# privacy-scaling-explorations/snark-verifier

Measured on AMD Instinct MI355X. Metric: BN254 G1 MSM points/sec at 2^20, higher is better.
Workload: dtype i32x9 (254-bit Montgomery Fq as 9 x 29-bit limbs on the integer VALU); 1 GPU; BN254 G1 Pippenger MSM, 2^20 random points/scalars per GPU, inputs resident in HBM, affine result (configs[1]); points_per_gpu=1048576, points_per_kernel_launch=1048576, window_bits=default, msms_in_flight=264

## Files before the change

snark-verifier_amd/csrc/msm_api.hip:

```cpp
#include <stdlib.h>
#include <algorithm>
#include "ctx.hpp"
#include "../../include/snarkv_pallas.h"

namespace snarkv {

bool pip_chunk_pipeline(size_t n, int window_bits, bool is_lane, size_t* chunk) {
  const size_t c = (size_t)1 << 20;
  const char* e = getenv("SNARKV_PIP_SPLIT");
  const int mode = e ? atoi(e) : 1;
  const size_t min_chunks = mode == 2 ? 2 : 3;
  if (chunk) *chunk = c;
  return SNARKV_CHUNK_PIPELINE && mode != 0 && (n + c - 1) / c >= min_chunks && window_bits == 0 && !is_lane;
}

int launch_msm_pippenger_auto(snarkv_ctx* ctx, const void* d_s, const void* d_p, size_t n, int window_bits, void* d_out,
                              bool partial_out) {
  size_t kChunk = 0;
  const bool split = pip_chunk_pipeline(n, window_bits, ctx->is_lane, &kChunk);
  const size_t chunks = (n + kChunk - 1) / kChunk;
  ctx->last_split_workers = 0;
  ctx->last_many_jobs = 0;
  if (!split) return launch_msm_pippenger(ctx, d_s, d_p, n, window_bits, d_out, partial_out);
  SNARKV_TRY(ctx_lanes(ctx));
  const bool tm = ctx->stage_timing;
  if (tm && !ctx->ev_ready) {
    for (int i = 0; i <= SNARKV_PIP_STAGES; ++i) SNARKV_HIP(hipEventCreate(&ctx->ev[i]));
    ctx->ev_ready = true;
  }
  if (tm) SNARKV_HIP(hipEventRecord(ctx->ev[0], ctx->stream));
  uint32_t c = 0, windows = 0, bpw = 0;
  SNARKV_TRY(pip_geometry(kChunk, 0, &c, &windows, &bpw));
  const size_t nb = (size_t)windows * bpw, grid_bytes = nb * SNARKV_G1_PARTIAL_BYTES;
  const int kWorkers = 2;
  void *grid[3], *tmp[3];
  bool started[3] = {false, false, false};
  for (int w = 0; w < kWorkers; ++w) {
    SNARKV_TRY(ctx_reserve(ctx->sub[w], SLOT_MGPU_GRID, grid_bytes, &grid[w]));
    SNARKV_TRY(ctx_reserve(ctx->sub[w], SLOT_MGPU_RECV, grid_bytes, &tmp[w]));
  }
  SNARKV_TRY(ctx_lanes_fork(ctx));
  for (size_t k = 0; k < chunks; ++k) {
    size_t lo = k * kChunk, len = std::min(kChunk, n - lo);
    int w = (int)(k % kWorkers);
    snarkv_ctx* lane = ctx->sub[w];
    lane->mont = ctx->mont;
    lane->stage_timing = tm;
    SNARKV_TRY(launch_msm_pippenger(lane, (const char*)d_s + 32 * lo, (const char*)d_p + 64 * lo, len, (int)c, nullptr, false,
                                    started[w] ? tmp[w] : grid[w]));
    if (started[w]) SNARKV_TRY(launch_buckets_add(lane, grid[w], tmp[w], nb));
    started[w] = true;
  }
  for (int w = 0; w < kWorkers; ++w) ctx->sub[w]->stage_timing = false;
  SNARKV_TRY(ctx_lanes_join(ctx));
  for (int w = 1; w < kWorkers; ++w)
    if (started[w]) SNARKV_TRY(launch_buckets_add(ctx, grid[0], grid[w], nb));
  void* d_part;
  SNARKV_TRY(ctx_reserve(ctx, SLOT_SPLIT_PARTIALS, SNARKV_G1_PARTIAL_BYTES, &d_part));
  ctx->last_split_workers = kWorkers;
  int rc = SNARKV_OK;
  if (partial_out) {
    rc = launch_buckets_reduce(ctx, grid[0], c, 0, windows, d_out);
  } else {
    rc = launch_buckets_reduce(ctx, grid[0], c, 0, windows, d_part);
    if (rc == SNARKV_OK) rc = launch_fold_partials(ctx, d_part, 1, d_out, false);
  }
  if (tm && rc == SNARKV_OK) SNARKV_HIP(hipEventRecord(ctx->ev[SNARKV_PIP_STAGES - 1], ctx->stream));
  return rc;
}

int launch_msm_pippenger_many(snarkv_ctx* ctx, size_t count, const void* const* d_s, const void* const* d_p,
                              const size_t* n, int window_bits, void* d_out, bool partial_out, hipEvent_t* ready) {
  const size_t ostride = partial_out ? SNARKV_G1_PARTIAL_BYTES : 64;
  ctx->last_many_jobs = 0;
  ctx->last_split_workers = 0;
  if (count == 0) return SNARKV_OK;
  uint32_t c0 = 0, w0 = 0, b0 = 0;
  bool uniform = true, large = false;
  size_t nmax = 0, sig = count * 1000003u + (size_t)(uint32_t)window_bits;
  for (size_t i = 0; i < count; ++i) {
    if (n[i] == 0) return SNARKV_ERR_EMPTY;
    uint32_t c, w, b;
    SNARKV_TRY(pip_geometry(n[i], window_bits, &c, &w, &b));
    if (i == 0) c0 = c, w0 = w, b0 = b;
    uniform = uniform && c == c0;
    large = large || pip_chunk_pipeline(n[i], window_bits, false, nullptr);
    nmax = std::max(nmax, n[i]);
    sig = sig * 31 + n[i];
  }
  const char* em = getenv("SNARKV_MANY_MODE");
  if (count == 1 || large || (em && atoi(em) == 0) || ctx->is_lane) {
    for (size_t i = 0; i < count; ++i) {
      if (ready) SNARKV_HIP(hipStreamWaitEvent(ctx->stream, ready[i], 0));
      SNARKV_TRY(launch_msm_pippenger_auto(ctx, d_s[i], d_p[i], n[i], window_bits, (uint8_t*)d_out + ostride * i, partial_out));
    }
    return SNARKV_OK;
  }
  const size_t per_job = nmax * 600 + (size_t)w0 * b0 * SNARKV_G1_PARTIAL_BYTES * 2 + (1u << 20);
  size_t G = std::min<size_t>(count, SNARKV_MANY_MAX_JOBS);
  G = std::max<size_t>(1, std::min<size_t>(G, ((size_t)48 << 30) / per_job));
  if (const char* eg = getenv("SNARKV_MANY_JOBS")) G = std::max<size_t>(1, std::min<size_t>(G, (size_t)atoi(eg)));
  const size_t rounds = (count + G - 1) / G;
  G = (count + rounds - 1) / rounds;
  SNARKV_TRY(ctx_lanes(ctx));
  while ((size_t)ctx->njobs < G) {
    snarkv_ctx* j = nullptr;
    SNARKV_TRY(SNARKV_API(ctx_create)(ctx->device, (void*)ctx->stream, &j));
    j->is_lane = true;
    j->throughput_mode = true;
    SNARKV_HIP(hipEventCreateWithFlags(&j->sorted_ev, hipEventDisableTiming));
    j->sorted_ev_ready = true;
    ctx->jobs[ctx->njobs++] = j;
  }
  if (!ctx->hi_ready) {
    int least = 0, greatest = 0;
    SNARKV_HIP(hipDeviceGetStreamPriorityRange(&least, &greatest));
    for (int i = 0; i < 2; ++i) SNARKV_HIP(hipStreamCreateWithPriority(&ctx->hi_stream[i], hipStreamNonBlocking, greatest));
    for (int i = 0; i < 2; ++i) SNARKV_HIP(hipEventCreateWithFlags(&ctx->many_ev[i], hipEventDisableTiming));
    ctx->hi_ready = true;
  }
  const bool tm = ctx->stage_timing;
  if (tm && !ctx->ev_ready) {
    for (int i = 0; i <= SNARKV_PIP_STAGES; ++i) SNARKV_HIP(hipEventCreate(&ctx->ev[i]));
    ctx->ev_ready = true;
  }
  if (sig != ctx->many_sig) {
    SNARKV_HIP(hipDeviceSynchronize());
    ctx->many_sig = sig;
  }
  hipStream_t S[3] = {ctx->stream, ctx->sub[0]->stream, ctx->sub[1]->stream};
  constexpr int nS = 3;
  auto join_and_fork = [&]() -> int {
    for (int k = 0; k < 2; ++k) {
      SNARKV_HIP(hipEventRecord(ctx->many_ev[k], ctx->hi_stream[k]));
      SNARKV_HIP(hipStreamWaitEvent(ctx->stream, ctx->many_ev[k], 0));
    }
    for (int k = 0; k + 1 < nS; ++k) {
      SNARKV_HIP(hipEventRecord(ctx->sub_ev[k], S[k + 1]));
      SNARKV_HIP(hipStreamWaitEvent(ctx->stream, ctx->sub_ev[k], 0));
    }
    SNARKV_HIP(hipEventRecord(ctx->sub_ev[4], ctx->stream));
    for (int k = 0; k < 2; ++k) SNARKV_HIP(hipStreamWaitEvent(ctx->hi_stream[k], ctx->sub_ev[4], 0));
    for (int k = 0; k + 1 < nS; ++k) SNARKV_HIP(hipStreamWaitEvent(S[k + 1], ctx->sub_ev[4], 0));
    return SNARKV_OK;
  };
  void* d_grids = nullptr;
  const size_t grid_bytes = (size_t)w0 * b0 * SNARKV_G1_PARTIAL_BYTES;
  if (uniform) SNARKV_TRY(ctx_reserve(ctx, SLOT_MGPU_GRID, grid_bytes * G, &d_grids));
  if (tm) SNARKV_HIP(hipEventRecord(ctx->ev[0], ctx->stream));
  SNARKV_TRY(join_and_fork());
  for (size_t lo = 0; lo < count; lo += G) {
    const size_t hi = std::min(count, lo + G);
    const bool last = hi == count;
    for (size_t i = lo; i < hi; ++i) {
      snarkv_ctx* job = ctx->jobs[i - lo];
      job->mont = ctx->mont;
      job->stage_timing = tm && last;
      void* grid = uniform ? (uint8_t*)d_grids + grid_bytes * (i - lo) : nullptr;
      hipStream_t sa = ctx->hi_stream[(i - lo) % 2], sb = S[(i - lo) % nS];
      if (ready) SNARKV_HIP(hipStreamWaitEvent(sa, ready[i], 0));
      SNARKV_TRY(launch_msm_pippenger_phases(job, sa, PIP_PHASE_SORT, d_s[i], d_p[i], n[i], window_bits, nullptr, false,
                                             nullptr, grid));
      SNARKV_HIP(hipEventRecord(job->sorted_ev, sa));
      SNARKV_HIP(hipStreamWaitEvent(sb, job->sorted_ev, 0));
      SNARKV_TRY(launch_msm_pippenger_phases(job, sb, PIP_PHASE_ACC, d_s[i], d_p[i], n[i], window_bits, nullptr, false,
                                             nullptr, grid));
      if (!uniform)
        SNARKV_TRY(launch_msm_pippenger_phases(job, sb, PIP_PHASE_TAIL, d_s[i], d_p[i], n[i], window_bits,
                                               (uint8_t*)d_out + ostride * i, partial_out, nullptr, nullptr));
      job->stage_timing = false;
    }
    SNARKV_TRY(join_and_fork());
    if (uniform) {
      SNARKV_TRY(launch_buckets_reduce_many(ctx, ctx->stream, d_grids, c0, w0, (uint32_t)(hi - lo),
                                            (uint8_t*)d_out + ostride * lo, partial_out));
      if (!last) SNARKV_TRY(join_and_fork());
    }
    if (last) ctx->last_many_jobs = (int)(hi - lo);
  }
  if (tm) SNARKV_HIP(hipEventRecord(ctx->ev[SNARKV_PIP_STAGES - 1], ctx->stream));
  return SNARKV_OK;
// ... 63 lines not shown
```

snark-verifier_amd/csrc/msm_pippenger.hip:

```cpp
#include <stdlib.h>
#include <string.h>
#include <algorithm>
#include <mutex>
#include <atomic>
#include "ctx.hpp"
#include "g1_29.h"
#include "fr29.h"
#ifndef SNARKV_GLV
#define SNARKV_GLV 1
#endif
#if SNARKV_GLV
#include "glv.h"
#endif

namespace snarkv {

#ifndef SNARKV_KRUN
#define SNARKV_KRUN 128
#endif
#ifndef SNARKV_KCHUNK
#define SNARKV_KCHUNK 8
#endif
#ifndef SNARKV_TILE_THREADS
#define SNARKV_TILE_THREADS 256
#endif
#ifndef SNARKV_SCATTER_ATTR
#define SNARKV_SCATTER_ATTR __attribute__((amdgpu_waves_per_eu(5)))
#endif
#ifndef SNARKV_L2_THREADS
#define SNARKV_L2_THREADS 512
#endif
#ifndef SNARKV_LEVEL2_ATTR
#define SNARKV_LEVEL2_ATTR
#endif
#ifndef SNARKV_PREP_THREADS
#define SNARKV_PREP_THREADS SNARKV_TILE_THREADS
#endif
#ifndef SNARKV_XCD_TILES
#define SNARKV_XCD_TILES 1
#endif
#ifndef SNARKV_TILE_BASE
#define SNARKV_TILE_BASE 2048
#endif
#ifndef SNARKV_ACC_WAVES
#define SNARKV_ACC_WAVES 3
#endif
#ifndef SNARKV_BPRIO
#define SNARKV_BPRIO 3
#endif
#define SNARKV_RAISE_PRIO() __builtin_amdgcn_s_setprio(SNARKV_BPRIO)

constexpr int kHalves = SNARKV_GLV ? 2 : 1;
constexpr int kDigitWords = SNARKV_GLV ? 4 : 8;
constexpr int kDigitBits = 32 * kDigitWords;
constexpr int kRun = SNARKV_KRUN;
#ifndef SNARKV_KRUN_THROUGHPUT
#define SNARKV_KRUN_THROUGHPUT 128
#endif
constexpr int kRunThroughput = SNARKV_KRUN_THROUGHPUT;
constexpr int kChunk = SNARKV_KCHUNK;
constexpr uint32_t kSortCap = 7168;
constexpr uint32_t kSortTarget = 3072;
constexpr uint32_t kMaxKeys = 16384;

struct PipParams {
  uint32_t n;
  int c;
  int W;
  uint32_t B;
  uint32_t nb;
  int low_bits;
  uint32_t SB;
  uint32_t nkeys;
  uint32_t nblk;
  uint32_t tile;
  uint32_t mstride;
  uint32_t w0;
  uint32_t krun;
  uint32_t wper;
  uint32_t chunk_log2;
  uint32_t mont;
};

__device__ __forceinline__ uint32_t half_bits(const uint32_t (&k)[kDigitWords], int lo, int c) {
  if (lo >= kDigitBits) return 0;
  int word = lo >> 5, sh = lo & 31;
  uint32_t w0 = 0u, w1 = 0u;
#pragma unroll
  for (int i = 0; i < kDigitWords; ++i) {
    w0 = word == i ? k[i] : w0;
    if (i > 0) w1 = word == i - 1 ? k[i] : w1;
  }
  uint64_t v = ((uint64_t)w1 << 32) | w0;
  return (uint32_t)(v >> sh) & ((1u << c) - 1u);
}

template <class F>
__device__ __forceinline__ void for_each_digit(const uint32_t (&k)[kDigitWords], uint32_t sgn, const PipParams& p, F emit) {
  uint32_t carry = 0;
  for (int w = 0; w < p.W; ++w) {
    uint32_t raw = half_bits(k, w * p.c, p.c) + carry;
    uint32_t neg = raw > p.B ? 1u : 0u;
    uint32_t d = neg ? ((1u << p.c) - raw) : raw;
    carry = neg;
    if (d != 0) emit((uint32_t)w * p.SB + ((d - 1) >> p.low_bits), (uint32_t)w * p.B + d - 1, neg ^ sgn);
  }
}
template <class F>
__device__ __forceinline__ void digit_of_window(const uint32_t (&k)[kDigitWords], uint32_t sgn, const PipParams& p, int w,
                                                F emit) {
  uint32_t carry = 0;
  for (int j = w - 1; j >= 0; --j) {
    uint32_t b = half_bits(k, j * p.c, p.c);
    if (b != p.B) {
      carry = b > p.B ? 1u : 0u;
      break;
    }
  }
  uint32_t raw = half_bits(k, w * p.c, p.c) + carry;
  uint32_t neg = raw > p.B ? 1u : 0u;
  uint32_t d = neg ? ((1u << p.c) - raw) : raw;
  if (d != 0) emit((uint32_t)w * p.SB + ((d - 1) >> p.low_bits), (uint32_t)w * p.B + d - 1, neg ^ sgn);
}
__device__ __forceinline__ uint32_t load_digit_words(const uint32_t* src, uint32_t (&k)[kDigitWords]) {
#pragma unroll
  for (int j = 0; j < kDigitWords; ++j) k[j] = src[j];
#if SNARKV_GLV
  uint32_t sgn = k[3] >> 31;
  k[3] &= 0x7FFFFFFFu;
  return sgn;
#else
  return 0u;
#endif
}
__device__ __forceinline__ uint32_t load_digit_source(const uint4* __restrict__ src, size_t v, uint32_t (&k)[kDigitWords]) {
  const uint4* s = src + v * (kDigitWords / 4);
#pragma unroll
  for (int j = 0; j < kDigitWords / 4; ++j) {
    uint4 q = s[j];
    k[4 * j] = q.x;
    k[4 * j + 1] = q.y;
    k[4 * j + 2] = q.z;
    k[4 * j + 3] = q.w;
  }
#if SNARKV_GLV
  uint32_t sgn = k[3] >> 31;
  k[3] &= 0x7FFFFFFFu;
  return sgn;
#else
  return 0u;
#endif
}

__device__ __forceinline__ uint32_t xcd_tile(uint32_t b, uint32_t nblk) {
#if SNARKV_XCD_TILES
  return (nblk & 7u) == 0 ? (b & 7u) * (nblk >> 3) + (b >> 3) : b;
#else
  return b;
#endif
}

__global__ void __launch_bounds__(SNARKV_PREP_THREADS)
    k_prepare(const uint32_t* __restrict__ scalars, const uint32_t* __restrict__ points,
              G1Packed* __restrict__ pts, uint4* __restrict__ glv, PipParams p, uint32_t* __restrict__ M) {
  SNARKV_RAISE_PRIO();
  extern __shared__ uint32_t lds[];
  for (uint32_t k = threadIdx.x; k < p.nkeys; k += blockDim.x) lds[k] = 0u;
  __syncthreads();
  const uint32_t tile = xcd_tile(blockIdx.x, p.nblk);
  uint32_t lo = tile * p.tile;
  uint32_t hi = lo + p.tile < p.n ? lo + p.tile : p.n;
  for (uint32_t i = lo + threadIdx.x; i < hi; i += blockDim.x) {
    const uint4* s = reinterpret_cast<const uint4*>(points + (size_t)i * 16);
    uint32_t w[16];
#pragma unroll
    for (int j = 0; j < 4; ++j) {
      uint4 v = s[j];
      w[4 * j] = v.x;
      w[4 * j + 1] = v.y;
      w[4 * j + 2] = v.z;
      w[4 * j + 3] = v.w;
    }
    G1Affine29 a = g1a29_from_words(w, p.mont != 0);
    bool ident = g1a29_is_identity(a);
    pts[kHalves * (size_t)i] = g1a29_pack(a);
    const uint4* ks = reinterpret_cast<const uint4*>(scalars + (size_t)i * 8);
    uint4 k0 = ks[0], k1 = ks[1];
    uint32_t k[8] = {k0.x, k0.y, k0.z, k0.w, k1.x, k1.y, k1.z, k1.w}, o[8];
    if (p.mont) {
      uint32_t kc[8];
      fr_words_from_mont256(k, kc);
#pragma unroll
      for (int j = 0; j < 8; ++j) k[j] = kc[j];
    }
#if SNARKV_GLV
    constexpr int32_t bl[9] = SNARKV_GLV_BETA29_LIMBS;
    Fq29 beta;
#pragma unroll
    for (int j = 0; j < 9; ++j) beta.v[j] = bl[j];
    a.x = fq29_canon_of_product(fq29_mul(a.x, beta));
    pts[2 * (size_t)i + 1] = g1a29_pack(a);
    glv_decompose(k, o);
#else
#pragma unroll
    for (int j = 0; j < 8; ++j) o[j] = k[j];
#endif
    if (ident) {
#pragma unroll
      for (int j = 0; j < 8; ++j) o[j] = 0;
    }
    glv[2 * (size_t)i] = make_uint4(o[0], o[1], o[2], o[3]);
    glv[2 * (size_t)i + 1] = make_uint4(o[4], o[5], o[6], o[7]);
#pragma unroll
    for (int h = 0; h < kHalves; ++h) {
      uint32_t d[kDigitWords];
      uint32_t sgn = load_digit_words(o + h * kDigitWords, d);
      for_each_digit(d, sgn, p, [&](uint32_t key, uint32_t, uint32_t) { atomicAdd(&lds[key], 1u); });
    }
  }
  __syncthreads();
  for (uint32_t k = threadIdx.x; k < p.nkeys; k += blockDim.x) M[(size_t)k * p.mstride + tile] = lds[k];
  if (blockIdx.x == 0 && p.mstride > p.nblk)
    for (uint32_t k = threadIdx.x; k < p.nkeys; k += blockDim.x) M[(size_t)k * p.mstride + p.nblk] = 0u;
}

constexpr uint32_t kStageScalars = SNARKV_TILE_BASE;
constexpr uint32_t kStageItems = kStageScalars / SNARKV_TILE_THREADS;
static_assert(kStageScalars % SNARKV_TILE_THREADS == 0, "a staged tile gives every lane the same number of scalars");
__global__ void __launch_bounds__(SNARKV_TILE_THREADS) SNARKV_SCATTER_ATTR
    k_sort_scatter_staged(const uint4* __restrict__ glv, PipParams p, const uint32_t* __restrict__ M,
                          uint2* __restrict__ tmp) {
  SNARKV_RAISE_PRIO();
  extern __shared__ uint32_t lds[];
  uint32_t* gbase = lds;
  uint32_t* cnt = lds + p.SB;
  uint32_t* off = lds + 2 * p.SB;
  uint32_t* wsum = lds + 3 * p.SB;
  uint2* stage = reinterpret_cast<uint2*>(lds + 3 * p.SB + 16 + (p.SB & 1u));
  const uint32_t tid = threadIdx.x, lane = tid & 63u, wave = tid >> 6;
  const uint32_t tile = xcd_tile(blockIdx.x, p.nblk);
  const uint32_t lo = tile * kStageScalars;
  const uint32_t hi = lo + kStageScalars < p.n ? lo + kStageScalars : p.n;
  const uint32_t per = (p.SB + SNARKV_TILE_THREADS - 1) / SNARKV_TILE_THREADS;
  for (int w = 0; w < p.W; ++w) {
    for (uint32_t k = tid; k < p.SB; k += blockDim.x) {
      gbase[k] = M[((size_t)w * p.SB + k) * p.mstride + tile];
      cnt[k] = 0u;
    }
    __syncthreads();
    uint32_t ebkt[kStageItems * kHalves], erank[kStageItems * kHalves], eneg = 0u;
#pragma unroll
    for (uint32_t j = 0; j < kStageItems; ++j) {
      const uint32_t i = lo + tid + j * SNARKV_TILE_THREADS;
#pragma unroll
      for (uint32_t h = 0; h < (uint32_t)kHalves; ++h) {
        const uint32_t e = j * kHalves + h;
        ebkt[e] = 0xFFFFFFFFu;
        if (i < hi) {
          uint32_t d[kDigitWords];
          uint32_t sgn = load_digit_source(glv, (size_t)kHalves * i + h, d);
          digit_of_window(d, sgn, p, w, [&](uint32_t key, uint32_t bucket, uint32_t neg) {
            ebkt[e] = bucket - (uint32_t)w * p.B;
            eneg |= neg << e;
            erank[e] = atomicAdd(&cnt[key - (uint32_t)w * p.SB], 1u);
          });
        }
      }
    }
    __syncthreads();
    uint32_t mine = 0;
    for (uint32_t k = tid * per; k < (tid + 1) * per && k < p.SB; ++k) mine += cnt[k];
    uint32_t incl = mine;
#pragma unroll
    for (int d = 1; d < 64; d <<= 1) {
      uint32_t up = __shfl_up(incl, d, 64);
      if ((int)lane >= d) incl += up;
    }
    if (lane == 63) wsum[wave] = incl;
    __syncthreads();
    uint32_t run = incl - mine;
    for (uint32_t q = 0; q < wave; ++q) run += wsum[q];
    for (uint32_t k = tid * per; k < (tid + 1) * per && k < p.SB; ++k) {
      off[k] = run;
      run += cnt[k];
    }
    __syncthreads();
#pragma unroll
    for (uint32_t e = 0; e < kStageItems * kHalves; ++e)
      if (ebkt[e] != 0xFFFFFFFFu) {
        const uint32_t v = kHalves * (lo + tid + (e / kHalves) * SNARKV_TILE_THREADS) + (e % kHalves);
        stage[off[ebkt[e] >> p.low_bits] + erank[e]] = make_uint2(ebkt[e] + (uint32_t)w * p.B, v | (((eneg >> e) & 1u) << 31));
      }
    __syncthreads();
    const uint32_t total = off[p.SB - 1] + cnt[p.SB - 1];
    for (uint32_t idx = tid; idx < total; idx += blockDim.x) {
      const uint2 e = stage[idx];
      const uint32_t key = (e.x - (uint32_t)w * p.B) >> p.low_bits;
      tmp[gbase[key] + (idx - off[key])] = e;
    }
    __syncthreads();
  }
}

__global__ void __launch_bounds__(256) k_scan_local(uint32_t* __restrict__ data, uint32_t* __restrict__ blocksum,
                                                    uint32_t nb) {
  SNARKV_RAISE_PRIO();
  __shared__ uint32_t sh[256];
  uint32_t base = blockIdx.x * 1024 + threadIdx.x * 4;
  uint32_t v[4], s = 0;
#pragma unroll
  for (int j = 0; j < 4; ++j) {
    v[j] = (base + j < nb) ? data[base + j] : 0;
    s += v[j];
  }
  sh[threadIdx.x] = s;
  __syncthreads();
  for (uint32_t off = 1; off < 256; off <<= 1) {
    uint32_t t = (threadIdx.x >= off) ? sh[threadIdx.x - off] : 0;
    __syncthreads();
    sh[threadIdx.x] += t;
    __syncthreads();
  }
  uint32_t excl = sh[threadIdx.x] - s;
#pragma unroll
  for (int j = 0; j < 4; ++j) {
    if (base + j < nb) data[base + j] = excl;
    excl += v[j];
  }
  if (threadIdx.x == 255) blocksum[blockIdx.x] = sh[255];
}

__global__ void __launch_bounds__(1024) k_scan_blocksums(uint32_t* __restrict__ blocksum, uint32_t nblocks,
                                                         uint32_t* __restrict__ total_out) {
  SNARKV_RAISE_PRIO();
  __shared__ uint32_t sh[1024];
  __shared__ uint32_t running;
  if (threadIdx.x == 0) running = 0;
  __syncthreads();
  for (uint32_t base = 0; base < nblocks; base += 1024) {
    uint32_t idx = base + threadIdx.x;
    uint32_t v = idx < nblocks ? blocksum[idx] : 0;
    sh[threadIdx.x] = v;
    __syncthreads();
    for (uint32_t off = 1; off < 1024; off <<= 1) {
      uint32_t t = (threadIdx.x >= off) ? sh[threadIdx.x - off] : 0;
      __syncthreads();
      sh[threadIdx.x] += t;
      __syncthreads();
// ... 475 lines not shown
                     (uint32_t*)d_out64, partial_out ? 1 : 0, ctx->mont ? 1u : 0u);
  SNARKV_HIP(hipGetLastError());
  return SNARKV_OK;
}

static int default_window_bits(size_t n) {
  int best = 2;
  double best_cost = 0;
  for (int c = 2; c <= 22; ++c) {
    const int W = (kDigitBits + c - 1) / c;
    const int top = kDigitBits - 1 - (W - 1) * c;
    double cost = (double)kHalves * (double)n * W * 10.0 + (double)W * (double)(1u << (c - 1)) * 30.0;
    if (top < c - 3) cost *= 1.6;
    if (c == 2 || cost < best_cost) best = c, best_cost = cost;
  }
  return best;
}

static int balance_window_bits(int c) {
  int W = (kDigitBits + c - 1) / c;
  return (kDigitBits + W - 1) / W;
}

static uint32_t latency_run_length(uint64_t entries) {
  auto waves = [&](uint64_t run) { return (entries + 64 * run - 1) / (64 * run); };
  if (waves(16) <= 4608) return waves(16) >= 2048 ? 16u : 32u;
  if (waves(32) <= 4608) return 32u;
  return (uint32_t)kRun;
}
static_assert(kRun >= 32 && kRun <= (int)kMaxPiece && kRunThroughput >= 16 && kRunThroughput <= (int)kMaxPiece,
              "piece caps fit the schedule's LDS rows");

int launch_msm_pippenger(snarkv_ctx* ctx, const void* d_scalars, const void* d_points, size_t n, int window_bits,
                         void* d_out, bool partial_out, void* d_buckets_out) {
  return launch_msm_pippenger_phases(ctx, ctx->stream, PIP_PHASE_ALL, d_scalars, d_points, n, window_bits, d_out,
                                     partial_out, d_buckets_out, nullptr);
}

int launch_msm_pippenger_phases(snarkv_ctx* ctx, hipStream_t st, int phases, const void* d_scalars, const void* d_points,
                                size_t n, int window_bits, void* d_out, bool partial_out, void* d_buckets_out,
                                void* d_grid) {
  PipParams p;
  p.w0 = 0;
  p.wper = 0;
  p.chunk_log2 = (uint32_t)kLog2Chunk;
  p.mont = ctx->mont ? 1u : 0u;
  p.n = (uint32_t)n;
  p.c = window_bits > 0 ? window_bits : balance_window_bits(default_window_bits(n));
  if (p.c < 2) p.c = 2;
  if (p.c > 22) p.c = 22;
  p.W = (kDigitBits + p.c - 1) / p.c;
  p.B = 1u << (p.c - 1);
  p.nb = (uint32_t)p.W * p.B;
  int high = p.c - 1 > 10 ? p.c - 1 - 10 : 0;
  while (high < p.c - 1 && ((kHalves * n) >> (high + 1)) >= kSortTarget && ((uint64_t)p.W << (high + 1)) <= kMaxKeys) ++high;
  p.low_bits = (p.c - 1) - high;
  p.SB = p.B >> p.low_bits;
  p.nkeys = (uint32_t)p.W * p.SB;
  p.tile = SNARKV_TILE_BASE;
  static_assert(kStageItems * kHalves <= 32, "a staged lane keeps one sign bit per entry in a 32-bit word");
  const size_t lds_staged = ((size_t)3 * p.SB + 16 + (p.SB & 1u)) * 4 + (size_t)kStageScalars * kHalves * 8;
  p.nblk = (uint32_t)((n + p.tile - 1) / p.tile);
  p.mstride = p.nblk | 1u;
  uint64_t max_entries = (uint64_t)kHalves * (uint64_t)n * (uint64_t)p.W;
  if (n == 0 || max_entries >= 0xFFFFFFFFull || n >= 0x40000000ull) {
    set_last_error("pippenger: n=%zu out of range", n);
    return SNARKV_ERR_LENGTH;
  }
  if ((size_t)p.nkeys * 4 > 65536 || lds_staged > 96 * 1024) {
    set_last_error("pippenger: key table too large (nkeys=%u)", p.nkeys);
    return SNARKV_ERR_LENGTH;
  }
  p.krun = ctx->throughput_mode ? (uint32_t)kRunThroughput : latency_run_length(max_entries);
  const uint32_t max_pieces = (uint32_t)std::min<uint64_t>((uint64_t)p.nb + max_entries / p.krun, 0xFFFFFFFFull - 63);
  const uint32_t split_slots = (uint32_t)(max_entries / p.krun) + 1;
  const uint32_t nsb = (p.nb + kSchedBuckets - 1) / kSchedBuckets;
  const uint32_t hcount = sched_rows(p.krun) * nsb;
  const uint32_t hscan_blocks = (hcount + 1023) / 1024;
  uint32_t mcount = p.nkeys * p.mstride;
  uint32_t scan_blocks = (mcount + 1023) / 1024;
  uint32_t chunks_per_window = (p.B + kChunk - 1) / kChunk;
  uint32_t blocks_per_window = (chunks_per_window + 63) / 64;

  void *d_pts, *d_glv, *d_counts, *d_offsets, *d_M, *d_blocksum, *d_entries, *d_tmp, *d_pieces, *d_hist, *d_parts,
      *d_buckets, *d_wave, *d_shift, *d_misc, *d_lists;
  SNARKV_TRY(ctx_reserve(ctx, SLOT_POINTS_MONT, kHalves * n * sizeof(G1Packed), &d_pts));
  SNARKV_TRY(ctx_reserve(ctx, SLOT_GLV, n * 32, &d_glv));
  SNARKV_TRY(ctx_reserve(ctx, SLOT_COUNTS, (size_t)p.nb * 4, &d_counts));
  SNARKV_TRY(ctx_reserve(ctx, SLOT_OFFSETS, (size_t)p.nb * 4, &d_offsets));
  SNARKV_TRY(ctx_reserve(ctx, SLOT_CURSOR, (size_t)mcount * 4, &d_M));
  SNARKV_TRY(ctx_reserve(ctx, SLOT_BLOCKSUMS, (size_t)std::max(scan_blocks, hscan_blocks) * 4 + 64, &d_blocksum));
  SNARKV_TRY(ctx_reserve(ctx, SLOT_ENTRIES, max_entries * 8, &d_entries));
  SNARKV_TRY(ctx_reserve(ctx, SLOT_SORT_TMP, max_entries * 8, &d_tmp));
  SNARKV_TRY(ctx_reserve(ctx, SLOT_PIECES, (size_t)max_pieces * sizeof(uint4), &d_pieces));
  SNARKV_TRY(ctx_reserve(ctx, SLOT_PIECE_HIST, (size_t)hcount * 4, &d_hist));
  SNARKV_TRY(ctx_reserve(ctx, SLOT_SPLIT_PARTS, (size_t)split_slots * 2 * sizeof(G1Xyzz29), &d_parts));
  if (d_grid) d_buckets = d_grid;
  else SNARKV_TRY(ctx_reserve(ctx, SLOT_BUCKETS, (size_t)p.nb * sizeof(G1Xyzz29), &d_buckets));
  SNARKV_TRY(ctx_reserve(ctx, SLOT_CHUNK_PARTIALS, 2 * (size_t)blocks_per_window * p.W * sizeof(G1Xyzz29), &d_wave));
  SNARKV_TRY(ctx_reserve(ctx, SLOT_SHIFTED, (size_t)p.W * sizeof(G1Xyzz29), &d_shift));
  SNARKV_TRY(ctx_reserve(ctx, SLOT_MISC, 64, &d_misc));
  SNARKV_TRY(ctx_reserve(ctx, SLOT_FIX_LISTS, (size_t)p.nb * 3 * 4, &d_lists));
  uint32_t* d_total = (uint32_t*)d_misc;
  uint32_t* d_small = (uint32_t*)d_lists, *d_bigl = d_small + p.nb, *d_deg = d_bigl + p.nb;
  const uint32_t* d_npieces = (const uint32_t*)d_hist + (size_t)(p.krun + 1) * nsb;

  const bool tm = ctx->stage_timing && phases == PIP_PHASE_ALL;
  const bool tm_acc = ctx->stage_timing && phases == PIP_PHASE_ACC;
  int evi = 0;
#define STAGE_MARK()                                         \
  do {                                                       \
    if (tm) SNARKV_HIP(hipEventRecord(ctx->ev[evi++], st));  \
  } while (0)
  if ((tm || tm_acc) && !ctx->ev_ready) {
    for (int i = 0; i <= SNARKV_PIP_STAGES; ++i) SNARKV_HIP(hipEventCreate(&ctx->ev[i]));
    ctx->ev_ready = true;
  }
  STAGE_MARK();
  if (phases & PIP_PHASE_SORT) {
    hipLaunchKernelGGL(k_prepare, dim3(p.nblk), dim3(SNARKV_PREP_THREADS), (size_t)p.nkeys * 4, st, (const uint32_t*)d_scalars,
                       (const uint32_t*)d_points, (G1Packed*)d_pts, (uint4*)d_glv, p, (uint32_t*)d_M);
    STAGE_MARK();
    hipLaunchKernelGGL(k_scan_local, dim3(scan_blocks), dim3(256), 0, st, (uint32_t*)d_M, (uint32_t*)d_blocksum, mcount);
    hipLaunchKernelGGL(k_scan_blocksums, dim3(1), dim3(1024), 0, st, (uint32_t*)d_blocksum, scan_blocks, d_total);
    hipLaunchKernelGGL(k_scan_add, dim3(scan_blocks), dim3(256), 0, st, (uint32_t*)d_M, (const uint32_t*)d_blocksum,
                       mcount);
    STAGE_MARK();
    static std::atomic<uint64_t> attr_set{0};
    const uint64_t bit = 1ull << (ctx->device & 63);
    if (!(attr_set.load(std::memory_order_relaxed) & bit)) {
      SNARKV_HIP(hipFuncSetAttribute(reinterpret_cast<const void*>(k_sort_scatter_staged),
                                     hipFuncAttributeMaxDynamicSharedMemorySize, 96 * 1024));
      attr_set.fetch_or(bit, std::memory_order_relaxed);
    }
    hipLaunchKernelGGL(k_sort_scatter_staged, dim3(p.nblk), dim3(SNARKV_TILE_THREADS), lds_staged, st, (const uint4*)d_glv,
                       p, (const uint32_t*)d_M, (uint2*)d_tmp);
    const uint32_t nbins_l2 = 1u << p.low_bits;
    const size_t lds2 = ((size_t)nbins_l2 + SNARKV_L2_THREADS + 1) * 4 + (size_t)kSortCap * 8;
    hipLaunchKernelGGL(k_sort_level2, dim3(p.nkeys), dim3(SNARKV_L2_THREADS), lds2, st, (const uint2*)d_tmp, (const uint32_t*)d_M,
                       d_total, p, (uint2*)d_entries, (uint32_t*)d_counts, (uint32_t*)d_offsets);
    hipLaunchKernelGGL(k_piece_hist, dim3(nsb), dim3(256), 0, st, (const uint32_t*)d_counts, p, nsb, (uint32_t*)d_hist,
                       d_total);
    hipLaunchKernelGGL(k_scan_local, dim3(hscan_blocks), dim3(256), 0, st, (uint32_t*)d_hist, (uint32_t*)d_blocksum, hcount);
    hipLaunchKernelGGL(k_scan_blocksums, dim3(1), dim3(1024), 0, st, (uint32_t*)d_blocksum, hscan_blocks, d_total + 6);
    hipLaunchKernelGGL(k_scan_add, dim3(hscan_blocks), dim3(256), 0, st, (uint32_t*)d_hist, (const uint32_t*)d_blocksum,
                       hcount);
    hipLaunchKernelGGL(k_piece_emit, dim3(nsb), dim3(256), 0, st, (const uint32_t*)d_counts, (const uint32_t*)d_offsets, p,
                       nsb, (const uint32_t*)d_hist, split_slots, (uint4*)d_pieces, d_small, d_bigl);
  }
  STAGE_MARK();
  if (tm_acc) SNARKV_HIP(hipEventRecord(ctx->ev[3], st));
  if (phases & PIP_PHASE_ACC)
    hipLaunchKernelGGL(k_accumulate, dim3((max_pieces + 63) / 64), dim3(64), 0, st, (const uint4*)d_pieces, d_npieces,
                       (const uint32_t*)d_total, (const uint2*)d_entries, (const G1Packed*)d_pts, (G1Xyzz29*)d_buckets,
                       (G1Xyzz29*)d_parts, 2 * split_slots, d_total + 4, d_deg, p);
  STAGE_MARK();
  if (tm_acc) SNARKV_HIP(hipEventRecord(ctx->ev[4], st));
  if (phases & PIP_PHASE_ACC) {
    const uint64_t split_bound = std::min<uint64_t>(p.nb, max_entries / (p.krun + 1) + 1);
    const uint32_t fix_grid = (uint32_t)std::min<uint64_t>((split_bound + 255) / 256, kFixGrid);
    hipLaunchKernelGGL(k_fixup, dim3(fix_grid), dim3(256), 0, st, (const uint32_t*)d_counts, (const uint32_t*)d_offsets,
                       (const uint2*)d_entries, (const G1Packed*)d_pts, (const G1Xyzz29*)d_parts, split_slots,
                       (G1Xyzz29*)d_buckets, (const uint32_t*)d_hist, nsb, (const uint32_t*)d_total,
                       (const uint32_t*)d_small, (const uint32_t*)d_bigl, (const uint32_t*)d_deg, p);
    if (tm_acc) SNARKV_HIP(hipEventRecord(ctx->ev[5], st));
  }
  STAGE_MARK();
  if (d_buckets_out) {
    if (phases & PIP_PHASE_ACC)
      SNARKV_HIP(hipMemcpyAsync(d_buckets_out, d_buckets, (size_t)p.nb * sizeof(G1Xyzz29), hipMemcpyDeviceToDevice, st));
    SNARKV_HIP(hipGetLastError());
    return SNARKV_OK;
  }
  if (phases & PIP_PHASE_TAIL)
    hipLaunchKernelGGL(k_bucket_reduce, dim3(blocks_per_window * p.W), dim3(64), 0, st, (const G1Xyzz29*)d_buckets,
                       (G1Xyzz29*)d_wave, p, chunks_per_window, blocks_per_window);
  STAGE_MARK();
  if (phases & PIP_PHASE_TAIL)
    hipLaunchKernelGGL(k_shift_windows, dim3(p.W), dim3(64), 0, st, (const G1Xyzz29*)d_wave, (G1Xyzz29*)d_shift, p,
                       blocks_per_window);
  STAGE_MARK();
  if (phases & PIP_PHASE_TAIL)
    hipLaunchKernelGGL(k_final, dim3(1), dim3(64), 0, st, (const G1Xyzz29*)d_shift, (uint32_t)p.W, (uint32_t*)d_out,
                       partial_out ? 1 : 0, p.mont);
  STAGE_MARK();
#undef STAGE_MARK
  SNARKV_HIP(hipGetLastError());
  return SNARKV_OK;
}

int pip_geometry(size_t n_total, int window_bits, uint32_t* c, uint32_t* windows, uint32_t* buckets_per_window) {
  int cc = window_bits > 0 ? window_bits : balance_window_bits(default_window_bits(n_total));
  if (cc < 2) cc = 2;
  if (cc > 22) cc = 22;
  *c = (uint32_t)cc;
  *windows = (uint32_t)((kDigitBits + cc - 1) / cc);
  *buckets_per_window = 1u << (cc - 1);
  return SNARKV_OK;
}

__global__ void __launch_bounds__(256) k_buckets_add(G1Xyzz29* __restrict__ dst, const G1Xyzz29* __restrict__ src, uint32_t count) {
  SNARKV_RAISE_PRIO();
  uint32_t i = blockIdx.x * blockDim.x + threadIdx.x;
  if (i >= count) return;
  G1Xyzz29 a = dst[i];
  xyzz29_add_careful(a, src[i]);
  dst[i] = xyzz29_sanitize(a);
}

int launch_buckets_add(snarkv_ctx* ctx, void* d_dst, const void* d_src, size_t count) {
  hipLaunchKernelGGL(k_buckets_add, dim3((uint32_t)((count + 255) / 256)), dim3(256), 0, ctx->stream, (G1Xyzz29*)d_dst,
                     (const G1Xyzz29*)d_src, (uint32_t)count);
  SNARKV_HIP(hipGetLastError());
  return SNARKV_OK;
}

int launch_buckets_reduce(snarkv_ctx* ctx, const void* d_buckets, uint32_t c, uint32_t w0, uint32_t wcount,
                          void* d_partial) {
// ... 79 lines not shown
```

Baseline: 806.2 million points/s.

## Precompute signed window digits in prepare and store per-window digit planes

The prepare kernel now computes the signed-digit recoding once per scalar and writes a per-window plane of packed digit records (magnitude plus sign bit), with a specialised unrolled path for 16-bit windows. The scatter kernel then reads one small record per window instead of reloading the full GLV scalar halves and rescanning lower windows for the carry. This removes redundant digit recomputation and large scalar reloads in the sort scatter, at the cost of more global writes in prepare and a differently sized scratch buffer. The per-job memory estimate is raised to match.

```diff
diff --git a/snark-verifier_amd/csrc/msm_api.hip b/snark-verifier_amd/csrc/msm_api.hip
--- a/snark-verifier_amd/csrc/msm_api.hip
+++ b/snark-verifier_amd/csrc/msm_api.hip
@@ -96,7 +96,7 @@
     }
     return SNARKV_OK;
   }
-  const size_t per_job = nmax * 600 + (size_t)w0 * b0 * SNARKV_G1_PARTIAL_BYTES * 2 + (1u << 20);
+  const size_t per_job = nmax * 632 + (size_t)w0 * b0 * SNARKV_G1_PARTIAL_BYTES * 2 + (1u << 20);
   size_t G = std::min<size_t>(count, SNARKV_MANY_MAX_JOBS);
   G = std::max<size_t>(1, std::min<size_t>(G, ((size_t)48 << 30) / per_job));
   if (const char* eg = getenv("SNARKV_MANY_JOBS")) G = std::max<size_t>(1, std::min<size_t>(G, (size_t)atoi(eg)));
diff --git a/snark-verifier_amd/csrc/msm_pippenger.hip b/snark-verifier_amd/csrc/msm_pippenger.hip
--- a/snark-verifier_amd/csrc/msm_pippenger.hip
+++ b/snark-verifier_amd/csrc/msm_pippenger.hip
@@ -12,6 +12,7 @@
 #if SNARKV_GLV
 #include "glv.h"
 #endif
+#include "pip_digits.h"
 
 namespace snarkv {
 
@@ -82,46 +83,9 @@
   uint32_t mont;
 };
 
-__device__ __forceinline__ uint32_t half_bits(const uint32_t (&k)[kDigitWords], int lo, int c) {
-  if (lo >= kDigitBits) return 0;
-  int word = lo >> 5, sh = lo & 31;
-  uint32_t w0 = 0u, w1 = 0u;
-#pragma unroll
-  for (int i = 0; i < kDigitWords; ++i) {
-    w0 = word == i ? k[i] : w0;
-    if (i > 0) w1 = word == i - 1 ? k[i] : w1;
-  }
-  uint64_t v = ((uint64_t)w1 << 32) | w0;
-  return (uint32_t)(v >> sh) & ((1u << c) - 1u);
-}
-
-template <class F>
-__device__ __forceinline__ void for_each_digit(const uint32_t (&k)[kDigitWords], uint32_t sgn, const PipParams& p, F emit) {
-  uint32_t carry = 0;
-  for (int w = 0; w < p.W; ++w) {
-    uint32_t raw = half_bits(k, w * p.c, p.c) + carry;
-    uint32_t neg = raw > p.B ? 1u : 0u;
-    uint32_t d = neg ? ((1u << p.c) - raw) : raw;
-    carry = neg;
-    if (d != 0) emit((uint32_t)w * p.SB + ((d - 1) >> p.low_bits), (uint32_t)w * p.B + d - 1, neg ^ sgn);
-  }
-}
-template <class F>
-__device__ __forceinline__ void digit_of_window(const uint32_t (&k)[kDigitWords], uint32_t sgn, const PipParams& p, int w,
-                                                F emit) {
-  uint32_t carry = 0;
-  for (int j = w - 1; j >= 0; --j) {
-    uint32_t b = half_bits(k, j * p.c, p.c);
-    if (b != p.B) {
-      carry = b > p.B ? 1u : 0u;
-      break;
-    }
-  }
-  uint32_t raw = half_bits(k, w * p.c, p.c) + carry;
-  uint32_t neg = raw > p.B ? 1u : 0u;
-  uint32_t d = neg ? ((1u << p.c) - raw) : raw;
-  if (d != 0) emit((uint32_t)w * p.SB + ((d - 1) >> p.low_bits), (uint32_t)w * p.B + d - 1, neg ^ sgn);
-}
+#ifndef SNARKV_DIGITS_GENERIC
+#define SNARKV_DIGITS_GENERIC 0
+#endif
 __device__ __forceinline__ uint32_t load_digit_words(const uint32_t* src, uint32_t (&k)[kDigitWords]) {
 #pragma unroll
   for (int j = 0; j < kDigitWords; ++j) k[j] = src[j];
@@ -133,24 +97,15 @@
   return 0u;
 #endif
 }
-__device__ __forceinline__ uint32_t load_digit_source(const uint4* __restrict__ src, size_t v, uint32_t (&k)[kDigitWords]) {
-  const uint4* s = src + v * (kDigitWords / 4);
-#pragma unroll
-  for (int j = 0; j < kDigitWords / 4; ++j) {
-    uint4 q = s[j];
-    k[4 * j] = q.x;
-    k[4 * j + 1] = q.y;
-    k[4 * j + 2] = q.z;
-    k[4 * j + 3] = q.w;
-  }
 #if SNARKV_GLV
-  uint32_t sgn = k[3] >> 31;
-  k[3] &= 0x7FFFFFFFu;
-  return sgn;
+typedef uint2 DigitPair;
+__device__ __forceinline__ DigitPair digit_pair(const uint32_t (&r)[kHalves]) { return make_uint2(r[0], r[1]); }
+__device__ __forceinline__ void digit_unpair(DigitPair q, uint32_t (&r)[kHalves]) { r[0] = q.x, r[1] = q.y; }
 #else
-  return 0u;
-#endif
-}
+typedef uint32_t DigitPair;
+__device__ __forceinline__ DigitPair digit_pair(const uint32_t (&r)[kHalves]) { return r[0]; }
+__device__ __forceinline__ void digit_unpair(DigitPair q, uint32_t (&r)[kHalves]) { r[0] = q; }
+#endif
 
 __device__ __forceinline__ uint32_t xcd_tile(uint32_t b, uint32_t nblk) {
 #if SNARKV_XCD_TILES
@@ -162,7 +117,7 @@
 
 __global__ void __launch_bounds__(SNARKV_PREP_THREADS)
     k_prepare(const uint32_t* __restrict__ scalars, const uint32_t* __restrict__ points,
-              G1Packed* __restrict__ pts, uint4* __restrict__ glv, PipParams p, uint32_t* __restrict__ M) {
+              G1Packed* __restrict__ pts, uint32_t* __restrict__ dig, PipParams p, uint32_t* __restrict__ M) {
   SNARKV_RAISE_PRIO();
   extern __shared__ uint32_t lds[];
   for (uint32_t k = threadIdx.x; k < p.nkeys; k += blockDim.x) lds[k] = 0u;
@@ -209,13 +164,35 @@
 #pragma unroll
       for (int j = 0; j < 8; ++j) o[j] = 0;
     }
-    glv[2 * (size_t)i] = make_uint4(o[0], o[1], o[2], o[3]);
-    glv[2 * (size_t)i + 1] = make_uint4(o[4], o[5], o[6], o[7]);
+    uint32_t d[kHalves][kDigitWords], sgn[kHalves], carry[kHalves];
 #pragma unroll
     for (int h = 0; h < kHalves; ++h) {
-      uint32_t d[kDigitWords];
-      uint32_t sgn = load_digit_words(o + h * kDigitWords, d);
-      for_each_digit(d, sgn, p, [&](uint32_t key, uint32_t, uint32_t) { atomicAdd(&lds[key], 1u); });
+      sgn[h] = load_digit_words(o + h * kDigitWords, d[h]);
+      carry[h] = 0u;
+    }
+    DigitPair* plane = reinterpret_cast<DigitPair*>(dig) + i;
+    auto window = [&](int w, const uint32_t (&rec)[kHalves]) {
+      plane[(size_t)w * p.n] = digit_pair(rec);
+#pragma unroll
+      for (int h = 0; h < kHalves; ++h)
+        if (rec[h]) atomicAdd(&lds[(uint32_t)w * p.SB + (((rec[h] & kDigitMag) - 1u) >> p.low_bits)], 1u);
+    };
+    if (!SNARKV_DIGITS_GENERIC && p.c == 16) {
+#pragma unroll
+      for (int w = 0; w < kDigitBits / 16; ++w)
+        if (w < p.W) {
+          uint32_t rec[kHalves];
+#pragma unroll
+          for (int h = 0; h < kHalves; ++h) rec[h] = digit_step16<kDigitWords>(d[h], sgn[h], w, carry[h]);
+          window(w, rec);
+        }
+    } else {
+      for (int w = 0; w < p.W; ++w) {
+        uint32_t rec[kHalves];
+#pragma unroll
+        for (int h = 0; h < kHalves; ++h) rec[h] = digit_step<kDigitWords>(d[h], sgn[h], w, p.c, carry[h]);
+        window(w, rec);
+      }
     }
   }
   __syncthreads();
@@ -228,7 +205,7 @@
 constexpr uint32_t kStageItems = kStageScalars / SNARKV_TILE_THREADS;
 static_assert(kStageScalars % SNARKV_TILE_THREADS == 0, "a staged tile gives every lane the same number of scalars");
 __global__ void __launch_bounds__(SNARKV_TILE_THREADS) SNARKV_SCATTER_ATTR
-    k_sort_scatter_staged(const uint4* __restrict__ glv, PipParams p, const uint32_t* __restrict__ M,
+    k_sort_scatter_staged(const uint32_t* __restrict__ dig, PipParams p, const uint32_t* __restrict__ M,
                           uint2* __restrict__ tmp) {
   SNARKV_RAISE_PRIO();
   extern __shared__ uint32_t lds[];
@@ -249,21 +226,22 @@
     }
     __syncthreads();
     uint32_t ebkt[kStageItems * kHalves], erank[kStageItems * kHalves], eneg = 0u;
+    const DigitPair* plane = reinterpret_cast<const DigitPair*>(dig) + (size_t)w * p.n;
 #pragma unroll
     for (uint32_t j = 0; j < kStageItems; ++j) {
       const uint32_t i = lo + tid + j * SNARKV_TILE_THREADS;
+      uint32_t rec[kHalves];
+#pragma unroll
+      for (int h = 0; h < kHalves; ++h) rec[h] = 0u;
+      if (i < hi) digit_unpair(plane[i], rec);
 #pragma unroll
       for (uint32_t h = 0; h < (uint32_t)kHalves; ++h) {
         const uint32_t e = j * kHalves + h;
         ebkt[e] = 0xFFFFFFFFu;
-        if (i < hi) {
-          uint32_t d[kDigitWords];
-          uint32_t sgn = load_digit_source(glv, (size_t)kHalves * i + h, d);
-          digit_of_window(d, sgn, p, w, [&](uint32_t key, uint32_t bucket, uint32_t neg) {
-            ebkt[e] = bucket - (uint32_t)w * p.B;
-            eneg |= neg << e;
-            erank[e] = atomicAdd(&cnt[key - (uint32_t)w * p.SB], 1u);
-          });
+        if (rec[h]) {
+          ebkt[e] = (rec[h] & kDigitMag) - 1u;
+          eneg |= (rec[h] >> 31) << e;
+          erank[e] = atomicAdd(&cnt[ebkt[e] >> p.low_bits], 1u);
         }
       }
     }
@@ -905,10 +883,10 @@
   uint32_t chunks_per_window = (p.B + kChunk - 1) / kChunk;
   uint32_t blocks_per_window = (chunks_per_window + 63) / 64;
 
-  void *d_pts, *d_glv, *d_counts, *d_offsets, *d_M, *d_blocksum, *d_entries, *d_tmp, *d_pieces, *d_hist, *d_parts,
+  void *d_pts, *d_dig, *d_counts, *d_offsets, *d_M, *d_blocksum, *d_entries, *d_tmp, *d_pieces, *d_hist, *d_parts,
       *d_buckets, *d_wave, *d_shift, *d_misc, *d_lists;
   SNARKV_TRY(ctx_reserve(ctx, SLOT_POINTS_MONT, kHalves * n * sizeof(G1Packed), &d_pts));
-  SNARKV_TRY(ctx_reserve(ctx, SLOT_GLV, n * 32, &d_glv));
+  SNARKV_TRY(ctx_reserve(ctx, SLOT_GLV, max_entries * 4, &d_dig));
   SNARKV_TRY(ctx_reserve(ctx, SLOT_COUNTS, (size_t)p.nb * 4, &d_counts));
   SNARKV_TRY(ctx_reserve(ctx, SLOT_OFFSETS, (size_t)p.nb * 4, &d_offsets));
   SNARKV_TRY(ctx_reserve(ctx, SLOT_CURSOR, (size_t)mcount * 4, &d_M));
@@ -942,7 +920,7 @@
   STAGE_MARK();
   if (phases & PIP_PHASE_SORT) {
     hipLaunchKernelGGL(k_prepare, dim3(p.nblk), dim3(SNARKV_PREP_THREADS), (size_t)p.nkeys * 4, st, (const uint32_t*)d_scalars,
-                       (const uint32_t*)d_points, (G1Packed*)d_pts, (uint4*)d_glv, p, (uint32_t*)d_M);
+                       (const uint32_t*)d_points, (G1Packed*)d_pts, (uint32_t*)d_dig, p, (uint32_t*)d_M);
     STAGE_MARK();
     hipLaunchKernelGGL(k_scan_local, dim3(scan_blocks), dim3(256), 0, st, (uint32_t*)d_M, (uint32_t*)d_blocksum, mcount);
     hipLaunchKernelGGL(k_scan_blocksums, dim3(1), dim3(1024), 0, st, (uint32_t*)d_blocksum, scan_blocks, d_total);
@@ -956,7 +934,7 @@
                                      hipFuncAttributeMaxDynamicSharedMemorySize, 96 * 1024));
       attr_set.fetch_or(bit, std::memory_order_relaxed);
     }
-    hipLaunchKernelGGL(k_sort_scatter_staged, dim3(p.nblk), dim3(SNARKV_TILE_THREADS), lds_staged, st, (const uint4*)d_glv,
+    hipLaunchKernelGGL(k_sort_scatter_staged, dim3(p.nblk), dim3(SNARKV_TILE_THREADS), lds_staged, st, (const uint32_t*)d_dig,
                        p, (const uint32_t*)d_M, (uint2*)d_tmp);
     const uint32_t nbins_l2 = 1u << p.low_bits;
     const size_t lds2 = ((size_t)nbins_l2 + SNARKV_L2_THREADS + 1) * 4 + (size_t)kSortCap * 8;
diff --git a/snark-verifier_amd/csrc/pip_digits.h b/snark-verifier_amd/csrc/pip_digits.h
--- /dev/null
+++ b/snark-verifier_amd/csrc/pip_digits.h
@@ -0,0 +1,59 @@
+#pragma once
+#include <stdint.h>
+#include "fq.h"
+
+namespace snarkv {
+
+constexpr uint32_t kDigitNeg = 0x80000000u;
+constexpr uint32_t kDigitMag = 0x7FFFFFFFu;
+
+template <int NW>
+SNARKV_HD uint32_t digit_bits(const uint32_t (&k)[NW], int lo, int c) {
+  if (lo >= 32 * NW) return 0;
+  int word = lo >> 5, sh = lo & 31;
+  uint32_t w0 = 0u, w1 = 0u;
+#pragma unroll
+  for (int i = 0; i < NW; ++i) {
+    w0 = word == i ? k[i] : w0;
+    if (i > 0) w1 = word == i - 1 ? k[i] : w1;
+  }
+  uint64_t v = ((uint64_t)w1 << 32) | w0;
+  return (uint32_t)(v >> sh) & ((1u << c) - 1u);
+}
+
+template <int NW>
+SNARKV_HD uint32_t digit_field16(const uint32_t (&k)[NW], int w) {
+  return (w & 1) ? k[w >> 1] >> 16 : k[w >> 1] & 0xFFFFu;
+}
+
+SNARKV_HD uint32_t digit_record(uint32_t bits, int c, uint32_t sgn, uint32_t& carry) {
+  const uint32_t raw = bits + carry, B = 1u << (c - 1);
+  const uint32_t neg = raw > B ? 1u : 0u;
+  const uint32_t d = neg ? (1u << c) - raw : raw;
+  carry = neg;
+  return d ? d | ((neg ^ sgn) << 31) : 0u;
+}
+
+template <int NW>
+SNARKV_HD uint32_t digit_step(const uint32_t (&k)[NW], uint32_t sgn, int w, int c, uint32_t& carry) {
+  return digit_record(digit_bits<NW>(k, w * c, c), c, sgn, carry);
+}
+template <int NW>
+SNARKV_HD uint32_t digit_step16(const uint32_t (&k)[NW], uint32_t sgn, int w, uint32_t& carry) {
+  return digit_record(digit_field16<NW>(k, w), 16, sgn, carry);
+}
+
+template <int NW>
+SNARKV_HD void digit_records(const uint32_t (&k)[NW], uint32_t sgn, int c, int W, uint32_t* rec) {
+  uint32_t carry = 0;
+  for (int w = 0; w < W; ++w) rec[w] = digit_step<NW>(k, sgn, w, c, carry);
+}
+template <int NW>
+SNARKV_HD void digit_records16(const uint32_t (&k)[NW], uint32_t sgn, int W, uint32_t* rec) {
+  uint32_t carry = 0;
+#pragma unroll
+  for (int w = 0; w < 2 * NW; ++w)
+    if (w < W) rec[w] = digit_step16<NW>(k, sgn, w, carry);
+}
+
+}
```

After: 809.5 million points/s, median of 2. About the same (+0.4%).
